# kubernetes-sigs/lws

Hardware: AMD Instinct MI355X
Metric: replica-group time-to-ready + rollout p50; Llama-3-70B 1-leader/0-worker TP=1 (lower is better)
Workload: dtype bf16; 1 GPU; model=llama-3-70b, global_batch=32, seq_len=128, parallelism=tp1, group=1-leader/0-workers (size=1), replicas=1, collectives_staged=False, orchestrator=lws_amd in-process control plane

## Files before the change

### lws_amd/models/llama.py

```python
from __future__ import annotations

import math
from dataclasses import dataclass
import torch

from ..parallel.tp import ShardedLinear, all_gather_cat, all_reduce


@dataclass
class LlamaConfig:
    name: str = "llama"
    hidden_size: int = 4096
    intermediate_size: int = 14336
    num_layers: int = 32
    num_q_heads: int = 32
    num_kv_heads: int = 8
    head_dim: int = 128
    vocab_size: int = 128256
    rope_theta: float = 500000.0
    rms_eps: float = 1e-5
    max_position: int = 8192
    num_experts: int = 0
    num_experts_per_tok: int = 2

    @property
    def q_size(self) -> int:
        return self.num_q_heads * self.head_dim

    @property
    def kv_size(self) -> int:
        return self.num_kv_heads * self.head_dim

    def num_params(self) -> int:
        h, i, v = self.hidden_size, self.intermediate_size, self.vocab_size
        mlp = 3 * h * i
        if self.num_experts > 0:
            mlp = self.num_experts * 3 * h * i + h * self.num_experts
        per_layer = (h * self.q_size + 2 * h * self.kv_size + self.q_size * h
                     + mlp + 2 * h)
        return self.num_layers * per_layer + 2 * v * h + h


def llama3_8b() -> LlamaConfig:
    return LlamaConfig(name="llama-3-8b", hidden_size=4096,
                       intermediate_size=14336, num_layers=32, num_q_heads=32,
                       num_kv_heads=8, vocab_size=128256)


def llama3_70b() -> LlamaConfig:
    return LlamaConfig(name="llama-3-70b", hidden_size=8192,
                       intermediate_size=28672, num_layers=80, num_q_heads=64,
                       num_kv_heads=8, vocab_size=128256)


def mixtral_8x7b() -> LlamaConfig:
    return LlamaConfig(name="mixtral-8x7b", hidden_size=4096,
                       intermediate_size=14336, num_layers=32, num_q_heads=32,
                       num_kv_heads=8, vocab_size=32000, rope_theta=1e6,
                       num_experts=8, num_experts_per_tok=2)


def mixtral_tiny() -> LlamaConfig:
    return LlamaConfig(name="mixtral-tiny", hidden_size=256,
                       intermediate_size=512, num_layers=2, num_q_heads=8,
                       num_kv_heads=2, head_dim=128, vocab_size=1024,
                       max_position=2048, num_experts=4,
                       num_experts_per_tok=2)


def llama_tiny() -> LlamaConfig:
    return LlamaConfig(name="llama-tiny", hidden_size=256,
                       intermediate_size=512, num_layers=2, num_q_heads=8,
                       num_kv_heads=2, head_dim=128, vocab_size=1024,
                       max_position=2048)


def llama_tiny8() -> LlamaConfig:
    return LlamaConfig(name="llama-tiny8", hidden_size=256,
                       intermediate_size=512, num_layers=2, num_q_heads=8,
                       num_kv_heads=8, head_dim=128, vocab_size=1024,
                       max_position=2048)


def llama_tiny4() -> LlamaConfig:
    return LlamaConfig(name="llama-tiny4", hidden_size=256,
                       intermediate_size=512, num_layers=2, num_q_heads=8,
# ... 76 lines not shown
                w0 = lins[0].weight
                stacked = torch.empty(cfg.num_experts, *w0.shape,
                                      device=device, dtype=dtype)
                for i, lin in enumerate(lins):
                    lin.weight = stacked[i]
                return stacked
            self.experts_gate_up_w = stack(self.experts_gate_up)
            self.experts_down_w = stack(self.experts_down)
            self.gate_up = None
            self.down = None
        else:
            self.router = None
            self.gate_up = ShardedLinear(2 * cfg.intermediate_size, h, 0,
                                         tp_rank, tp_world, device, dtype)
            self.down = ShardedLinear(h, cfg.intermediate_size, 1, tp_rank,
                                      tp_world, device, dtype)
        self.input_norm = torch.empty(h, device=device, dtype=dtype)
        self.post_norm = torch.empty(h, device=device, dtype=dtype)
        self.q_slice = self.hq * d
        self.kv_slice = self.hkv * d

    def materialize(self, gen=None):
        lins = [self.qkv, self.o]
        if self.router is not None:
            self.router.normal_(0.0, 0.02, generator=gen)
            lins += self.experts_gate_up + self.experts_down
        else:
            lins += [self.gate_up, self.down]
        for lin in lins:
            lin.materialize(gen)
        self.input_norm.fill_(1.0)
        self.post_norm.fill_(1.0)

    @property
    def param_count(self) -> int:
        n = self.qkv.numel + self.o.numel
        n += self.input_norm.numel() + self.post_norm.numel()
        if self.router is not None:
            n += self.router.numel()
            n += sum(l.numel for l in self.experts_gate_up)
            n += sum(l.numel for l in self.experts_down)
        else:
            n += self.gate_up.numel + self.down.numel
        return n


class LlamaForCausalLM:
    def __init__(self, cfg: LlamaConfig, tp_rank: int = 0, tp_world: int = 1,
                 device: str = "cpu", dtype=torch.bfloat16,
                 pp_rank: int = 0, pp_world: int = 1):
        self.cfg = cfg
        self.tp_rank = tp_rank
        self.tp_world = tp_world
        self.pp_rank = pp_rank
        self.pp_world = pp_world
        assert tp_world == 1 or pp_world == 1, \
            "combined TP x PP grids are not supported"
        self.device = torch.device(device)
        self.dtype = dtype
        self._ops = _Ops(self.device)
        L, base, rem = cfg.num_layers, cfg.num_layers // pp_world, \
            cfg.num_layers % pp_world
        sizes = [base + (1 if r < rem else 0) for r in range(pp_world)]
        self.layer_offset = sum(sizes[:pp_rank])
        self.pp_first = pp_rank == 0
        self.pp_last = pp_rank == pp_world - 1
        self.layers = [LlamaLayer(cfg, tp_rank, tp_world, self.device, dtype)
                       for _ in range(sizes[pp_rank])]
        self.embed = torch.empty(cfg.vocab_size, cfg.hidden_size,
                                 device=self.device, dtype=dtype) \
            if self.pp_first else None
        self.final_norm = torch.empty(cfg.hidden_size, device=self.device,
                                      dtype=dtype) if self.pp_last else None
        self.lm_head = ShardedLinear(cfg.vocab_size, cfg.hidden_size, 0,
                                     tp_rank, tp_world, self.device, dtype) \
            if self.pp_last else None
        from lws_amd.ops import build_rope_table
        self.rope_table = build_rope_table(cfg.max_position, cfg.head_dim,
                                           cfg.rope_theta, device=self.device)
        self.scale = 1.0 / math.sqrt(cfg.head_dim)
        self._ar = all_reduce if tp_world > 1 else (lambda t: t)
        self._agc = all_gather_cat if tp_world > 1 \
            else (lambda t, dim=-1: t)

    def materialize(self, seed: int = 0) -> int:
        def gen_for(tag: int) -> torch.Generator:
            g = torch.Generator(device=self.device)
            g.manual_seed(seed * 1000003 + tag * 7919 + self.tp_rank)
            return g
        n = 0
        for i, layer in enumerate(self.layers):
            layer.materialize(gen_for(self.layer_offset + i))
            n += layer.param_count
        if self.embed is not None:
            self.embed.normal_(0.0, 0.02, generator=gen_for(500009))
            n += self.embed.numel()
        if self.final_norm is not None:
            self.final_norm.fill_(1.0)
            n += self.final_norm.numel()
        if self.lm_head is not None:
            self.lm_head.materialize(gen_for(600011))
            n += self.lm_head.numel
        return n

    def quantize_fp8(self) -> None:
        for layer in self.layers:
            lins = [layer.qkv, layer.o]
            if layer.router is None:
                lins += [layer.gate_up, layer.down]
            for lin in lins:
                lin.quantize_fp8()
            if layer.router is not None:
                for name, lins in (
                        ("experts_gate_up_w", layer.experts_gate_up),
                        ("experts_down_w", layer.experts_down)):
                    w = getattr(layer, name)
                    sc = (w.abs().amax(dim=2).float() / 448.0) \
                        .clamp(min=1e-8).contiguous()
                    w8 = (w.float() / sc[:, :, None]).clamp(-448.0, 448.0) \
                        .to(torch.float8_e4m3fn).contiguous()
                    setattr(layer, name + "8", w8)
                    setattr(layer, name + "_scale", sc)
                    setattr(layer, name, None)
                    for e, lin in enumerate(lins):
                        lin.weight_fp8 = w8[e]
                        lin.scale_fp8 = sc[e]
                        lin.weight = None
        if self.lm_head is not None:
            self.lm_head.quantize_fp8()

    def kv_cache_spec(self) -> tuple[int, int]:
        return len(self.layers), self.layers[0].hkv

    def _rmsnorm(self, x, w):
        if self._ops.is_gpu:
            return self._ops.ops.rmsnorm(x, w, self.cfg.rms_eps)
        return self._ops.ref.rmsnorm_ref(x, w, self.cfg.rms_eps)

    def _fused_add_rmsnorm(self, x, residual, w):
        if self._ops.is_gpu:
            self._ops.ops.fused_add_rmsnorm(x, residual, w, self.cfg.rms_eps)
            return x, residual
        out, new_res = self._ops.ref.fused_add_rmsnorm_ref(
            x, residual, w, self.cfg.rms_eps)
        return out, new_res

    def _silu_mul(self, gu):
        if self._ops.is_gpu:
            return self._ops.ops.silu_mul(gu)
        return self._ops.ref.silu_mul_ref(gu)

    def _write_cache(self, k, v, k_cache, v_cache, slot_mapping):
        if self._ops.is_gpu:
            self._ops.ops.reshape_and_cache(k, v, k_cache, v_cache, slot_mapping)
            return
        page = k_cache.size(2)
        for t in range(k.size(0)):
            s = int(slot_mapping[t])
            if s < 0:
                continue
            k_cache[s // page, :, s % page] = k[t]
            v_cache[s // page, :, s % page] = v[t]

    def _qkv_views(self, qkv: torch.Tensor, layer, positions):
        d = self.cfg.head_dim
        if self._ops.is_gpu:
            q = qkv.narrow(-1, 0, layer.q_slice).unflatten(-1, (layer.hq, d))
            k = qkv.narrow(-1, layer.q_slice,
                           layer.kv_slice).unflatten(-1, (layer.hkv, d))
            v = qkv.narrow(-1, layer.q_slice + layer.kv_slice,
                           layer.kv_slice).unflatten(-1, (layer.hkv, d))
            self._ops.ops.rope(q, k, self.rope_table, positions,
                               layer.hq, layer.hkv)
            return q, k, v
        q, k, v = qkv.split([layer.q_slice, layer.kv_slice, layer.kv_slice],
                            dim=-1)
        q, k = self._ops.ref.rope_ref(q.contiguous(), k.contiguous(),
                                      self.rope_table, positions,
                                      layer.hq, layer.hkv)
        T = qkv.size(0)
        return (q.view(T, layer.hq, d), k.view(T, layer.hkv, d),
                v.contiguous().view(T, layer.hkv, d))

    def forward_prefill(self, batch: PrefillBatch, kv_caches) -> torch.Tensor:
        cfg = self.cfg
        if self.pp_first:
            x = self.embed[batch.input_ids]
            residual = None
        else:
            from ..parallel import pp as ppmod
            T = batch.input_ids.size(0)
            st = ppmod.recv_stage((2, T, cfg.hidden_size), self.dtype,
                                  self.device, self.pp_rank - 1)
            x, residual = st[0], st[1]
        for li, layer in enumerate(self.layers):
            if residual is None:
                residual = x
                h = self._rmsnorm(x, layer.input_norm)
            else:
                h, residual = self._fused_add_rmsnorm(x, residual,
                                                      layer.input_norm)
            qkv = layer.qkv(h)
            q, k, v = self._qkv_views(qkv, layer, batch.positions)
            k_cache, v_cache = kv_caches[li]
            self._write_cache(k, v, k_cache, v_cache, batch.slot_mapping)
            attn = self._prefill_attention(q, k, v, batch, layer,
                                           k_cache, v_cache)
            o = layer.o(attn)
            x = self._ar(o)
            h, residual = self._fused_add_rmsnorm(x, residual, layer.post_norm)
            x = self._ar(self._mlp(layer, h))
        B = len(batch.seq_starts) - 1
        if not self.pp_last:
            from ..parallel import pp as ppmod
            ppmod.send_stage(torch.stack([x, residual]), self.pp_rank + 1)
            return torch.zeros(B, self.cfg.hidden_size, device=self.device,
                               dtype=self.dtype)
        h, _ = self._fused_add_rmsnorm(x, residual, self.final_norm)
        last = torch.tensor([s - 1 for s in batch.seq_starts[1:]],
                            device=h.device, dtype=torch.long)
        return h[last]

    def _prefill_attention(self, q, k, v, batch: PrefillBatch, layer,
                           k_cache, v_cache):
        cfg = self.cfg
        d = cfg.head_dim
        kv_starts = batch.seq_starts
        q_offsets = None
        if batch.kv_row_idx is not None:
            k = k_cache.reshape(-1, d).index_select(
                0, batch.kv_row_idx).view(-1, layer.hkv, d)
            v = v_cache.reshape(-1, d).index_select(
                0, batch.kv_row_idx).view(-1, layer.hkv, d)
            kv_starts = batch.kv_starts
            q_offsets = batch.q_offsets
        if self._ops.is_gpu:
            return self._ops.ops.prefill_attention(
                q, k, v, batch.seq_starts, self.scale,
                kv_starts=kv_starts, q_offsets=q_offsets)
        T = q.size(0)
        out = torch.empty(T, layer.hq * d, device=q.device, dtype=q.dtype)
        G = layer.hq // layer.hkv
        offs = q_offsets or [0] * (len(batch.seq_starts) - 1)
        for i in range(len(batch.seq_starts) - 1):
            s0, s1 = batch.seq_starts[i], batch.seq_starts[i + 1]
            kv0, kv1 = kv_starts[i], kv_starts[i + 1]
            S, KV, off = s1 - s0, kv1 - kv0, offs[i]
            qs = q[s0:s1].transpose(0, 1)
            ks = k[kv0:kv1].transpose(0, 1)
            vs = v[kv0:kv1].transpose(0, 1)
            ks = ks.repeat_interleave(G, dim=0)
            vs = vs.repeat_interleave(G, dim=0)
            scores = (qs @ ks.transpose(-1, -2)).float() * self.scale
            cols = torch.arange(KV, device=q.device)
            rows = torch.arange(S, device=q.device)
            mask = torch.where(cols[None, :] > off + rows[:, None],
                               float("-inf"), 0.0)
            p = torch.softmax(scores + mask, dim=-1).to(q.dtype)
            o = (p @ vs).transpose(0, 1).reshape(S, layer.hq * d)
            out[s0:s1] = o
        return out

    def forward_decode(self, batch: DecodeBatch, kv_caches) -> torch.Tensor:
        cfg = self.cfg
        if self.pp_first:
            x = self.embed[batch.input_ids]
            residual = None
        else:
            from ..parallel import pp as ppmod
            B0 = batch.input_ids.size(0)
            st = ppmod.recv_stage((2, B0, cfg.hidden_size), self.dtype,
                                  self.device, self.pp_rank - 1)
            x, residual = st[0], st[1]
        fp8q = (self._ops.is_gpu and self.layers
                and getattr(self.layers[0].qkv, "weight_fp8", None)
                is not None and self.layers[0].router is None
                and x.size(0) <= 32 and cfg.hidden_size % 256 == 0
                and self.layers[0].down.weight_fp8.size(1) % 256 == 0)
        for li, layer in enumerate(self.layers):
            if fp8q:
                if residual is None:
                    residual = x
                    h8, hs = self._ops.ops.rmsnorm_fp8(x, layer.input_norm,
                                                       cfg.rms_eps)
                else:
                    h8, hs = self._ops.ops.fused_add_rmsnorm_fp8(
                        x, residual, layer.input_norm, cfg.rms_eps)
                qkv = layer.qkv.forward_q8(h8, hs)
            else:
                if residual is None:
                    residual = x
                    h = self._rmsnorm(x, layer.input_norm)
                else:
                    h, residual = self._fused_add_rmsnorm(x, residual,
                                                          layer.input_norm)
                qkv = layer.qkv(h)
            k_cache, v_cache = kv_caches[li]
            if self._ops.is_gpu:
                d = cfg.head_dim
                q = qkv.narrow(-1, 0, layer.q_slice) \
                    .unflatten(-1, (layer.hq, d))
                k = qkv.narrow(-1, layer.q_slice, layer.kv_slice) \
                    .unflatten(-1, (layer.hkv, d))
                vv = qkv.narrow(-1, layer.q_slice + layer.kv_slice,
                                layer.kv_slice).unflatten(-1, (layer.hkv, d))
                self._ops.ops.rope_and_cache(q, k, vv, self.rope_table,
                                             batch.positions, k_cache,
                                             v_cache, batch.slot_mapping)
            else:
                q, k, v = self._qkv_views(qkv, layer, batch.positions)
                self._write_cache(k, v, k_cache, v_cache,
                                  batch.slot_mapping)
            B = q.size(0)
            if self._ops.is_gpu:
                attn = self._ops.ops.paged_attention_decode(
                    q, k_cache, v_cache, batch.block_tables, batch.seq_lens,
                    self.scale)
            else:
                attn = self._ops.ref.paged_attention_decode_ref(
                    q.contiguous(), k_cache, v_cache, batch.block_tables,
                    batch.seq_lens, self.scale)
            o = layer.o(attn.view(B, layer.hq * cfg.head_dim))
            x = self._ar(o)
            if fp8q:
                h8, hs = self._ops.ops.fused_add_rmsnorm_fp8(
                    x, residual, layer.post_norm, cfg.rms_eps)
                gu = layer.gate_up.forward_q8(h8, hs)
                a8, ascale = self._ops.ops.silu_mul_fp8(gu)
                x = self._ar(layer.down.forward_q8(a8, ascale))
            else:
                h, residual = self._fused_add_rmsnorm(x, residual,
                                                      layer.post_norm)
                x = self._ar(self._mlp(layer, h))
        if not self.pp_last:
            from ..parallel import pp as ppmod
            ppmod.send_stage(torch.stack([x, residual]), self.pp_rank + 1)
            return torch.zeros_like(x)
        h, _ = self._fused_add_rmsnorm(x, residual, self.final_norm)
        return h

    def _mlp(self, layer, h: torch.Tensor) -> torch.Tensor:
        if layer.router is None:
            return layer.down(self._silu_mul(layer.gate_up(h)))
        cfg = self.cfg
        logits = (h.float() @ layer.router.float().t())
        weights, chosen = torch.topk(torch.softmax(logits, dim=-1),
                                     cfg.num_experts_per_tok, dim=-1)
        weights = weights / weights.sum(dim=-1, keepdim=True)
        out = torch.zeros_like(h)
        if self._ops.is_gpu and h.size(0) <= 32:
            E = cfg.num_experts
            T = h.size(0)
            tk = cfg.num_experts_per_tok
            flat = chosen.reshape(-1)
            oh = torch.nn.functional.one_hot(flat, E)
            ranks = oh.cumsum(0) - oh
            rank_sel = ranks.gather(1, flat.unsqueeze(1)).squeeze(1)
            dest = flat * T + rank_sel
            tok = torch.arange(T, device=h.device).repeat_interleave(tk)
            x_pad = torch.zeros(E * T, h.size(1), dtype=h.dtype,
                                device=h.device)
            x_pad.index_copy_(0, dest, h.index_select(0, tok))
# ... 37 lines not shown
```

### lws_amd/ops/__init__.py

```python
from __future__ import annotations

from pathlib import Path
from typing import Optional

import torch

_LIB = None
_LOAD_ERROR: Optional[str] = None


def _try_load() -> None:
    global _LIB, _LOAD_ERROR
    if _LIB is not None or _LOAD_ERROR is not None:
        return
    so = Path(__file__).resolve().parent / "_C.so"
    if not so.exists():
        _LOAD_ERROR = f"{so} not built (run python -m lws_amd.ops.build)"
        return
    try:
        torch.ops.load_library(str(so))
    except Exception:
        pass
    try:
        import importlib.util

        spec = importlib.util.spec_from_file_location("lws_amd_C", str(so))
        mod = importlib.util.module_from_spec(spec)
        spec.loader.exec_module(mod)
        _LIB = mod
    except Exception as e:
        _LOAD_ERROR = f"failed to load {so}: {e}"


def native_available() -> bool:
    _try_load()
    return _LIB is not None


def require_native():
    _try_load()
    if _LIB is None:
        raise RuntimeError(
            "lws_amd native kernels unavailable on a GPU host: "
            f"{_LOAD_ERROR}. Build with `python -m lws_amd.ops.build`.")
    return _LIB



def rmsnorm(x: torch.Tensor, weight: torch.Tensor, eps: float = 1e-5,
            out: Optional[torch.Tensor] = None) -> torch.Tensor:
    lib = require_native()
    if out is None:
        out = torch.empty_like(x)
    lib.rmsnorm(out, x, weight, eps)
    return out


def fused_add_rmsnorm(x: torch.Tensor, residual: torch.Tensor,
                      weight: torch.Tensor, eps: float = 1e-5) -> None:
    lib = require_native()
    lib.fused_add_rmsnorm(x, residual, weight, eps)


def silu_mul(gateup: torch.Tensor,
             out: Optional[torch.Tensor] = None) -> torch.Tensor:
    lib = require_native()
    shape = list(gateup.shape)
    shape[-1] //= 2
    if out is None:
        out = torch.empty(shape, dtype=gateup.dtype, device=gateup.device)
    lib.silu_mul(out, gateup)
    return out


def rope(q: torch.Tensor, k: torch.Tensor, cos_sin: torch.Tensor,
         positions: torch.Tensor, num_q_heads: int, num_kv_heads: int) -> None:
    lib = require_native()
    lib.rope(q, k, cos_sin, positions, num_q_heads, num_kv_heads)


def rope_and_cache(q, k, v, cos_sin, positions, k_cache, v_cache,
                   slot_mapping) -> None:
    lib = require_native()
    lib.rope_and_cache(q, k, v, cos_sin, positions, k_cache, v_cache,
                       slot_mapping)


def build_rope_table(max_pos: int, head_dim: int, theta: float = 10000.0,
                     device="cpu") -> torch.Tensor:
    half = head_dim // 2
    inv_freq = 1.0 / (theta ** (torch.arange(0, half, dtype=torch.float64) / half))
    pos = torch.arange(max_pos, dtype=torch.float64)
    ang = torch.outer(pos, inv_freq)
    table = torch.cat([torch.cos(ang), torch.sin(ang)], dim=-1).float()
    return table.to(device)


_PA_WS: dict = {}


def paged_attention_decode(q: torch.Tensor, k_cache: torch.Tensor,
                           v_cache: torch.Tensor, block_tables: torch.Tensor,
                           seq_lens: torch.Tensor, scale: float,
                           chunk_keys: Optional[int] = None,
                           workspace: Optional[tuple] = None,
                           out: Optional[torch.Tensor] = None) -> torch.Tensor:
    import os as _os

    lib = require_native()
    B, Hq, D = q.shape
    Hkv = k_cache.size(1)
    G = Hq // Hkv
    mfma = G in (4, 8, 16) and _os.environ.get("LWS_PA_MFMA", "1") != "0"
    max_len = int(block_tables.size(1)) * int(k_cache.size(2))
    if chunk_keys is None:
        if B * Hkv >= 256 and G == 1 and max_len <= 512:
            chunk_keys = ((max_len + 15) // 16) * 16
        else:
            if B * Hkv <= 64:
                if mfma:
                    target_chunks = max(1, min(8, -(-max_len // 64)))
                else:
                    target_chunks = min(16, (max_len + 31) // 32)
            else:
                target_chunks = max(1, min(4, -(-max_len // 96)))
            chunk_keys = -(-max_len // target_chunks)
            chunk_keys = ((chunk_keys + 15) // 16) * 16
    num_chunks = max(1, (max_len + chunk_keys - 1) // chunk_keys)
    if mfma:
        num_chunks *= 4
    if workspace is None:
        key = ("paws", B, Hkv, num_chunks, G, q.device.index)
        ws = _PA_WS.get(key)
        if ws is None:
            ws = (torch.empty((B, Hkv, num_chunks, G, D),
                              dtype=torch.float32, device=q.device),
                  torch.empty((B, Hkv, num_chunks, G, 2),
                              dtype=torch.float32, device=q.device))
            _PA_WS[key] = ws
        ws_acc, ws_ml = ws
    else:
        ws_acc, ws_ml = workspace
        num_chunks = ws_ml.size(2)
    if out is None:
        out = torch.empty_like(q)
    lib.paged_attention_decode(out, q, k_cache, v_cache, block_tables,
                               seq_lens, ws_acc, ws_ml, scale, chunk_keys)
    return out


def reshape_and_cache(k: torch.Tensor, v: torch.Tensor, k_cache: torch.Tensor,
                      v_cache: torch.Tensor, slot_mapping: torch.Tensor) -> None:
    lib = require_native()
    lib.reshape_and_cache(k, v, k_cache, v_cache, slot_mapping)


SKINNY_GEMM_MAX_M = 32
_SKINNY_WS: dict = {}


def skinny_gemm(x: torch.Tensor, w: torch.Tensor,
                out: Optional[torch.Tensor] = None) -> torch.Tensor:
    lib = require_native()
    grouped = x.dim() == 3
    E = x.size(0) if grouped else 1
    M, K = x.shape[-2], x.shape[-1]
    N = w.size(-2)
    if out is None:
        shape = (E, M, N) if grouped else (M, N)
        out = torch.empty(shape, dtype=x.dtype, device=x.device)
    import os
    target = int(os.environ.get("LWS_SG_TARGET", "256"))
    n_blocks = (N + 63) // 64
    split = min(max(1, target // max(1, n_blocks)), max(1, K // 128))
    k_slice = (K // split + 127) // 128 * 128
    grid_y = (K + k_slice - 1) // k_slice
    if grouped and E * n_blocks >= 256:
        grid_y = 1
    key = (grid_y, E, M, N, x.device.index)
    ws = _SKINNY_WS.get(key)
    if ws is None:
        ws = torch.empty(grid_y, E * M, N, dtype=torch.float32,
                         device=x.device)
        _SKINNY_WS[key] = ws
    lib.skinny_gemm(out, x, w, ws)
    return out


_SKINNY_FP8_BUFS: dict = {}


def skinny_gemm_fp8(x: torch.Tensor, w8: torch.Tensor, w_scale: torch.Tensor,
                    out: Optional[torch.Tensor] = None) -> torch.Tensor:
    lib = require_native()
    M, K = x.shape
    N = w8.size(0)
    if out is None:
        out = torch.empty(M, N, dtype=torch.bfloat16, device=x.device)
    import os
    target = int(os.environ.get("LWS_SG8_TARGET", "512"))
    ksub = int(os.environ.get("LWS_SG8_KSUB", "128"))
    rows = 32 if (os.environ.get("LWS_SG8_ROWS") == "32"
                  and ksub == 128) else 64
    n_blocks = (N + rows - 1) // rows
    split = min(max(1, target // max(1, n_blocks)), max(1, K // ksub))
    k_slice = (K // split + ksub - 1) // ksub * ksub
    grid_y = (K + k_slice - 1) // k_slice
    key = (grid_y, M, N, K, x.device.index)
    bufs = _SKINNY_FP8_BUFS.get(key)
    if bufs is None:
        bufs = (torch.empty(M, K, dtype=torch.float8_e4m3fn, device=x.device),
                torch.empty(M, dtype=torch.float32, device=x.device),
                torch.empty(grid_y, M, N, dtype=torch.float32,
                            device=x.device))
        _SKINNY_FP8_BUFS[key] = bufs
    x8, xs, ws = bufs
    lib.quant_fp8_rows(x8, xs, x.contiguous())
    lib.skinny_gemm_fp8(out, x8, xs, w8, w_scale, ws)
    return out


def skinny_gemm_fp8_grouped(x: torch.Tensor, w8: torch.Tensor,
                            w_scale: torch.Tensor,
                            out: Optional[torch.Tensor] = None
                            ) -> torch.Tensor:
    lib = require_native()
    E, M, K = x.shape
    N = w8.size(1)
    if out is None:
        out = torch.empty(E, M, N, dtype=torch.bfloat16, device=x.device)
    key = ("g8", E, M, N, K, x.device.index)
    bufs = _SKINNY_FP8_BUFS.get(key)
    if bufs is None:
        bufs = (torch.empty(E, M, K, dtype=torch.float8_e4m3fn,
                            device=x.device),
                torch.empty(E, M, dtype=torch.float32, device=x.device),
                torch.empty(1, M, N, dtype=torch.float32, device=x.device))
        _SKINNY_FP8_BUFS[key] = bufs
    x8, xs, ws = bufs
    lib.quant_fp8_rows(x8.view(E * M, K), xs.view(E * M), x.reshape(E * M, K))
    lib.skinny_gemm_fp8(out, x8, xs, w8, w_scale, ws)
    return out


def skinny_gemm_fp8_q(x8: torch.Tensor, xs: torch.Tensor, w8: torch.Tensor,
                      w_scale: torch.Tensor,
                      out: Optional[torch.Tensor] = None) -> torch.Tensor:
    lib = require_native()
    M, K = x8.shape
    N = w8.size(0)
    if out is None:
        out = torch.empty(M, N, dtype=torch.bfloat16, device=x8.device)
    import os
    target = int(os.environ.get("LWS_SG8_TARGET", "512"))
    ksub = int(os.environ.get("LWS_SG8_KSUB", "128"))
    rows = 32 if (os.environ.get("LWS_SG8_ROWS") == "32"
                  and ksub == 128) else 64
    n_blocks = (N + rows - 1) // rows
    split = min(max(1, target // max(1, n_blocks)), max(1, K // ksub))
    k_slice = (K // split + ksub - 1) // ksub * ksub
    grid_y = (K + k_slice - 1) // k_slice
    key = ("q8ws", grid_y, M, N, x8.device.index)
    ws = _SKINNY_FP8_BUFS.get(key)
    if ws is None:
        ws = torch.empty(grid_y, M, N, dtype=torch.float32, device=x8.device)
        _SKINNY_FP8_BUFS[key] = ws
    lib.skinny_gemm_fp8(out, x8, xs, w8, w_scale, ws)
    return out


_FP8_ACT_BUFS: dict = {}


def _fp8_act_buffers(rows: int, cols: int, device) -> tuple:
    key = (rows, cols, device.index if device.type == "cuda" else -1)
    bufs = _FP8_ACT_BUFS.get(key)
    if bufs is None:
        bufs = (torch.empty(rows, cols, dtype=torch.float8_e4m3fn,
                            device=device),
                torch.empty(rows, dtype=torch.float32, device=device))
        _FP8_ACT_BUFS[key] = bufs
    return bufs


def rmsnorm_fp8(x: torch.Tensor, weight: torch.Tensor,
                eps: float = 1e-5) -> tuple:
    lib = require_native()
    rows, D = x.shape[0], x.shape[-1]
    y8, ys = _fp8_act_buffers(rows, D, x.device)
    lib.rmsnorm_fp8(y8, ys, x.contiguous(), weight, eps)
    return y8, ys


def fused_add_rmsnorm_fp8(x: torch.Tensor, residual: torch.Tensor,
                          weight: torch.Tensor, eps: float = 1e-5) -> tuple:
    lib = require_native()
    rows, D = x.shape[0], x.shape[-1]
    y8, ys = _fp8_act_buffers(rows, D, x.device)
    lib.fused_add_rmsnorm_fp8(y8, ys, x.contiguous(), residual, weight, eps)
    return y8, ys


def silu_mul_fp8(gateup: torch.Tensor) -> tuple:
    lib = require_native()
    rows = gateup.shape[0]
    I = gateup.shape[-1] // 2
    a8, ascale = _fp8_act_buffers(rows, I, gateup.device)
    lib.silu_mul_fp8(a8, ascale, gateup.contiguous())
    return a8, ascale


def prefill_attention(q: torch.Tensor, k: torch.Tensor, v: torch.Tensor,
                      seq_starts: list, scale: float,
                      out: Optional[torch.Tensor] = None,
                      kv_starts: Optional[list] = None,
                      q_offsets: Optional[list] = None) -> torch.Tensor:
    lib = require_native()
    T, Hq, D = q.shape
    device = q.device
    B = len(seq_starts) - 1
    tile_seq, tile_q0 = [], []
    for i in range(B):
        S = seq_starts[i + 1] - seq_starts[i]
        for q0 in range(0, S, 64):
            tile_seq.append(i)
            tile_q0.append(q0)
    if kv_starts is None:
        kv_starts = seq_starts
    if q_offsets is None:
        q_offsets = [0] * B
    if out is None:
        out = torch.empty(T, Hq * D, dtype=q.dtype, device=device)
    lib.prefill_attention(
        out, q, k, v,
        torch.tensor(tile_seq, dtype=torch.int32, device=device),
        torch.tensor(tile_q0, dtype=torch.int32, device=device),
        torch.tensor(seq_starts, dtype=torch.int32, device=device),
        torch.tensor(kv_starts, dtype=torch.int32, device=device),
        torch.tensor(q_offsets, dtype=torch.int32, device=device), scale)
    return out
```

### lws_amd/ops/build.py

```python
from __future__ import annotations

import os
import shutil
import sys
from pathlib import Path

PKG_DIR = Path(__file__).resolve().parent
CSRC = PKG_DIR / "csrc"
SO_NAME = "_C.so"
SOURCES = ["norm_act.hip", "rope.hip", "paged_attention.hip",
           "skinny_gemm.hip", "skinny_gemm_fp8.hip", "prefill_attention.hip",
           "bindings.cpp"]


def _newest_source_mtime() -> float:
    return max((CSRC / s).stat().st_mtime for s in SOURCES) if CSRC.exists() else 0


def needs_build() -> bool:
    so = PKG_DIR / SO_NAME
    if not so.exists():
        return True
    return so.stat().st_mtime < _newest_source_mtime()


def build(verbose: bool = False, force: bool = False) -> Path:
    so_path = PKG_DIR / SO_NAME
    if not force and not needs_build():
        return so_path

    os.environ.setdefault("PYTORCH_ROCM_ARCH", "gfx950")
    from torch.utils.cpp_extension import load

    build_dir = PKG_DIR / "build"
    build_dir.mkdir(exist_ok=True)
    load(
        name="lws_amd_C",
        sources=[str(CSRC / s) for s in SOURCES],
        extra_cflags=["-O3", "-std=c++17"],
        extra_cuda_cflags=["-O3", "-std=c++17"],
        build_directory=str(build_dir),
        verbose=verbose,
        is_python_module=True,
        keep_intermediates=True,
    )
    built = build_dir / "lws_amd_C.so"
    if not built.exists():
        raise RuntimeError(f"extension build produced no {built}")
    shutil.copy2(built, so_path)
    return so_path


if __name__ == "__main__":
    p = build(verbose="-v" in sys.argv, force="-f" in sys.argv)
    print(f"built {p}")
```

### lws_amd/ops/csrc/bindings.cpp

```cpp
#include <torch/extension.h>

void rmsnorm(torch::Tensor out, torch::Tensor input, torch::Tensor weight,
             double eps);
void fused_add_rmsnorm(torch::Tensor x, torch::Tensor residual,
                       torch::Tensor weight, double eps);
void silu_mul(torch::Tensor out, torch::Tensor gateup);
void rmsnorm_fp8(torch::Tensor out8, torch::Tensor oscale,
                 torch::Tensor input, torch::Tensor weight, double eps);
void fused_add_rmsnorm_fp8(torch::Tensor out8, torch::Tensor oscale,
                           torch::Tensor x, torch::Tensor residual,
                           torch::Tensor weight, double eps);
void silu_mul_fp8(torch::Tensor out8, torch::Tensor oscale,
                  torch::Tensor gateup);
void rope(torch::Tensor q, torch::Tensor k, torch::Tensor cos_sin,
          torch::Tensor positions, long long num_q_heads,
          long long num_kv_heads);
void rope_and_cache(torch::Tensor q, torch::Tensor k, torch::Tensor v,
                    torch::Tensor cos_sin, torch::Tensor positions,
                    torch::Tensor k_cache, torch::Tensor v_cache,
                    torch::Tensor slot_mapping);
void paged_attention_decode(torch::Tensor out, torch::Tensor q,
                            torch::Tensor k_cache, torch::Tensor v_cache,
                            torch::Tensor block_tables, torch::Tensor seq_lens,
                            torch::Tensor ws_acc, torch::Tensor ws_ml,
                            double scale, long long chunk_keys);
void reshape_and_cache(torch::Tensor k, torch::Tensor v,
                       torch::Tensor k_cache, torch::Tensor v_cache,
                       torch::Tensor slot_mapping);
void skinny_gemm(torch::Tensor out, torch::Tensor x, torch::Tensor w,
                 torch::Tensor ws);
void skinny_gemm_fp8(torch::Tensor out, torch::Tensor x8, torch::Tensor xs,
                     torch::Tensor w8, torch::Tensor ws_n, torch::Tensor ws);
void quant_fp8_rows(torch::Tensor x8, torch::Tensor xs, torch::Tensor x);
void prefill_attention(torch::Tensor out, torch::Tensor q, torch::Tensor k,
                       torch::Tensor v, torch::Tensor tile_seq,
                       torch::Tensor tile_q0, torch::Tensor seq_starts,
                       torch::Tensor kv_starts, torch::Tensor q_offs,
                       double scale);

PYBIND11_MODULE(TORCH_EXTENSION_NAME, m) {
  m.def("rmsnorm", &rmsnorm, "RMSNorm (bf16, gfx950)");
  m.def("fused_add_rmsnorm", &fused_add_rmsnorm,
        "in-place residual add + RMSNorm (bf16, gfx950)");
  m.def("silu_mul", &silu_mul, "fused SiLU-gate multiply (bf16, gfx950)");
  m.def("rmsnorm_fp8", &rmsnorm_fp8,
        "RMSNorm with fused per-token e4m3 quantization epilogue");
  m.def("fused_add_rmsnorm_fp8", &fused_add_rmsnorm_fp8,
        "residual add + RMSNorm with fused e4m3 quantization epilogue");
  m.def("silu_mul_fp8", &silu_mul_fp8,
        "SiLU-gate multiply with fused e4m3 quantization epilogue");
  m.def("rope", &rope, "fused rotary embedding for q,k (bf16, gfx950)");
  m.def("rope_and_cache", &rope_and_cache,
        "rope on q in place + rotated k and v scattered into the paged "
        "KV cache (single decode launch)");
  m.def("paged_attention_decode", &paged_attention_decode,
        "GQA paged attention decode with flash-decoding chunk split");
  m.def("reshape_and_cache", &reshape_and_cache,
        "scatter new k/v into the paged KV cache");
  m.def("skinny_gemm", &skinny_gemm,
        "split-K MFMA GEMM for decode-shape projections (M<=32)");
  m.def("skinny_gemm_fp8", &skinny_gemm_fp8,
        "W8A8 e4m3 split-K MFMA GEMM for decode projections (M<=32)");
  m.def("quant_fp8_rows", &quant_fp8_rows,
        "per-token e4m3 activation quantization (bf16 -> fp8 + scales)");
  m.def("prefill_attention", &prefill_attention,
        "flash-style causal varlen prefill attention (GQA, gfx950)");
}
```

### lws_amd/parallel/tp.py

```python
from __future__ import annotations

import os
from dataclasses import dataclass
from typing import Optional

import torch
import torch.distributed as dist


@dataclass
class ParallelState:
    rank: int = 0
    world_size: int = 1
    local_rank: int = 0
    device: torch.device = torch.device("cpu")
    group: Optional[object] = None
    staged: bool = False

    @property
    def is_distributed(self) -> bool:
        return self.world_size > 1


_STATE = ParallelState()
# ... 32 lines not shown
    return _STATE


def all_reduce(t: torch.Tensor) -> torch.Tensor:
    if _STATE.is_distributed and dist.is_initialized():
        if _STATE.staged and t.is_cuda:
            host = t.detach().to("cpu")
            dist.all_reduce(host)
            t.copy_(host)
        else:
            dist.all_reduce(t)
    return t


def all_gather_cat(t: torch.Tensor, dim: int = -1) -> torch.Tensor:
    if not (_STATE.is_distributed and dist.is_initialized()):
        return t
    if _STATE.staged and t.is_cuda:
        host = t.detach().contiguous().to("cpu")
        parts = [torch.empty_like(host) for _ in range(_STATE.world_size)]
        dist.all_gather(parts, host)
        return torch.cat(parts, dim=dim).to(t.device)
    parts = [torch.empty_like(t) for _ in range(_STATE.world_size)]
    dist.all_gather(parts, t.contiguous())
    return torch.cat(parts, dim=dim)


def barrier() -> None:
    if _STATE.is_distributed and dist.is_initialized():
        dist.barrier()



class ShardedLinear:

    def __init__(self, out_features: int, in_features: int, shard_dim: int,
                 tp_rank: int, tp_world: int, device, dtype=torch.bfloat16):
        self.shard_dim = shard_dim
        if shard_dim == 0:
            assert out_features % tp_world == 0
            shape = (out_features // tp_world, in_features)
        else:
            assert in_features % tp_world == 0
            shape = (out_features, in_features // tp_world)
        self.weight = torch.empty(shape, device=device, dtype=dtype)
        self.weight_fp8: Optional[torch.Tensor] = None
        self.scale_fp8: Optional[torch.Tensor] = None
        self._ones: Optional[torch.Tensor] = None

    def materialize(self, generator: Optional[torch.Generator] = None,
                    std: float = 0.02) -> None:
        self.weight.normal_(0.0, std, generator=generator)

    def quantize_fp8(self) -> None:
        w = self.weight
        self.scale_fp8 = (w.abs().amax(dim=1).float() / 448.0) \
            .clamp(min=1e-8).contiguous()
        self.weight_fp8 = (w.float() / self.scale_fp8[:, None]).clamp(
            -448.0, 448.0).to(torch.float8_e4m3fn).contiguous()
        self.weight = None

    def __call__(self, x: torch.Tensor) -> torch.Tensor:
        if self.weight_fp8 is not None:
            M = x.size(0)
            if not x.is_cuda:
                wf = self.weight_fp8.float() * self.scale_fp8[:, None]
                return (x.float() @ wf.t()).to(torch.bfloat16)
            if x.dim() == 2 and M <= 32 and x.size(1) % 256 == 0:
                from .. import ops
                return ops.skinny_gemm_fp8(x, self.weight_fp8,
                                           self.scale_fp8)
            pad = (-M) % 16
            if pad:
                x = torch.nn.functional.pad(x, (0, 0, 0, pad))
            xs = (x.abs().amax().float() / 448.0).clamp(min=1e-8)
            x8 = (x.float() / xs).clamp(-448.0, 448.0).to(torch.float8_e4m3fn)
            if self._ones is None or self._ones.device != x.device:
                self._ones = torch.ones((), device=x.device)
            out = torch._scaled_mm(x8, self.weight_fp8.t(), scale_a=xs,
                                   scale_b=self._ones,
                                   out_dtype=torch.bfloat16)
            out = out * self.scale_fp8.to(torch.bfloat16)[None, :]
            return out[:M] if pad else out
        if x.is_cuda and x.dim() == 2 and x.size(0) <= 32 and \
                x.size(1) % 128 == 0 and self._skinny_wins():
            from .. import ops
            return ops.skinny_gemm(x.contiguous(), self.weight)
        return x @ self.weight.t()

    def _skinny_wins(self) -> bool:
        N, K = self.weight.shape
        if N * K <= 32 * 1024 * 1024:
            return True
        if K <= 4096:
            return True
        if K >= 16384 and N >= 8192:
            return True
        return False

    def forward_q8(self, x8: torch.Tensor, xs: torch.Tensor) -> torch.Tensor:
        from .. import ops
        return ops.skinny_gemm_fp8_q(x8, xs, self.weight_fp8, self.scale_fp8)

    @property
    def numel(self) -> int:
        w = self.weight if self.weight is not None else self.weight_fp8
        return w.numel()
```

Baseline: 287.1 ms.

## Move per-layer attention and MLP sequencing into native C++ block ops

Adds C++ entry points (decode_attn_block, prefill_attn_block, mlp_block) that run norm, QKV projection, rope/cache write, attention and output projection inside one native call per block. GEMM workspaces, the paged-attention plan and the prefill attention metadata tensors are now computed once per forward instead of once per layer. The aim is to cut Python dispatch and repeated host-to-device metadata tensor creation. It also adds a tightened N%16 condition for skinny GEMM and a new native path that has to stay numerically consistent with the Python path.

```diff
diff --git a/lws_amd/models/llama.py b/lws_amd/models/llama.py
--- a/lws_amd/models/llama.py
+++ b/lws_amd/models/llama.py
@@ -2,6 +2,8 @@
 
 import math
 from dataclasses import dataclass
+from typing import Optional
+
 import torch
 
 from ..parallel.tp import ShardedLinear, all_gather_cat, all_reduce
@@ -244,6 +246,19 @@
         self._ar = all_reduce if tp_world > 1 else (lambda t: t)
         self._agc = all_gather_cat if tp_world > 1 \
             else (lambda t, dim=-1: t)
+        self._native_blocks: Optional[bool] = None
+
+    @property
+    def native_blocks(self) -> bool:
+        if self._native_blocks is False:
+            return False
+        return (self._ops.is_gpu and bool(self.layers)
+                and self.layers[0].router is None
+                and self.layers[0].qkv.weight_fp8 is None)
+
+    @native_blocks.setter
+    def native_blocks(self, value: bool) -> None:
+        self._native_blocks = bool(value)
 
     def materialize(self, seed: int = 0) -> int:
         def gen_for(tag: int) -> torch.Generator:
@@ -355,7 +370,36 @@
             st = ppmod.recv_stage((2, T, cfg.hidden_size), self.dtype,
                                   self.device, self.pp_rank - 1)
             x, residual = st[0], st[1]
+        meta = None
+        if self._ops.is_gpu:
+            chunked = batch.kv_row_idx is not None
+            meta = self._ops.ops.prefill_attention_meta(
+                batch.seq_starts, batch.kv_starts if chunked else None,
+                batch.q_offsets if chunked else None, x.device)
+        native = self.native_blocks
+        if native:
+            lib = self._ops.ops.require_native()
+            T = x.size(0)
+            l0 = self.layers[0]
+            qkv_ws, o_ws = l0.qkv.plan(T), l0.o.plan(T)
+            gate_up_ws, down_ws = l0.gate_up.plan(T), l0.down.plan(T)
         for li, layer in enumerate(self.layers):
+            if native:
+                k_cache, v_cache = kv_caches[li]
+                o = lib.prefill_attn_block(
+                    x, residual, layer.input_norm, cfg.rms_eps,
+                    layer.qkv.weight, qkv_ws, layer.o.weight, o_ws,
+                    self.rope_table, batch.positions, k_cache, v_cache,
+                    batch.slot_mapping, batch.kv_row_idx, *meta, self.scale,
+                    layer.hq, layer.hkv)
+                if residual is None:
+                    residual = x
+                x = self._ar(o)
+                x = self._ar(lib.mlp_block(
+                    x, residual, layer.post_norm, cfg.rms_eps,
+                    layer.gate_up.weight, gate_up_ws, layer.down.weight,
+                    down_ws))
+                continue
             if residual is None:
                 residual = x
                 h = self._rmsnorm(x, layer.input_norm)
@@ -367,7 +411,7 @@
             k_cache, v_cache = kv_caches[li]
             self._write_cache(k, v, k_cache, v_cache, batch.slot_mapping)
             attn = self._prefill_attention(q, k, v, batch, layer,
-                                           k_cache, v_cache)
+                                           k_cache, v_cache, meta)
             o = layer.o(attn)
             x = self._ar(o)
             h, residual = self._fused_add_rmsnorm(x, residual, layer.post_norm)
@@ -384,7 +428,7 @@
         return h[last]
 
     def _prefill_attention(self, q, k, v, batch: PrefillBatch, layer,
-                           k_cache, v_cache):
+                           k_cache, v_cache, meta=None):
         cfg = self.cfg
         d = cfg.head_dim
         kv_starts = batch.seq_starts
@@ -399,7 +443,7 @@
         if self._ops.is_gpu:
             return self._ops.ops.prefill_attention(
                 q, k, v, batch.seq_starts, self.scale,
-                kv_starts=kv_starts, q_offsets=q_offsets)
+                kv_starts=kv_starts, q_offsets=q_offsets, meta=meta)
         T = q.size(0)
         out = torch.empty(T, layer.hq * d, device=q.device, dtype=q.dtype)
         G = layer.hq // layer.hkv
@@ -439,7 +483,35 @@
                 is not None and self.layers[0].router is None
                 and x.size(0) <= 32 and cfg.hidden_size % 256 == 0
                 and self.layers[0].down.weight_fp8.size(1) % 256 == 0)
+        native = self.native_blocks
+        if native:
+            lib = self._ops.ops.require_native()
+            B = x.size(0)
+            l0 = self.layers[0]
+            page_size = kv_caches[0][0].size(2)
+            chunk_keys, ws_acc, ws_ml = self._ops.ops.paged_attention_plan(
+                B, l0.hq, l0.hkv, cfg.head_dim,
+                int(batch.block_tables.size(1)) * int(page_size), x.device)
+            qkv_ws, o_ws = l0.qkv.plan(B), l0.o.plan(B)
+            gate_up_ws, down_ws = l0.gate_up.plan(B), l0.down.plan(B)
         for li, layer in enumerate(self.layers):
+            if native:
+                k_cache, v_cache = kv_caches[li]
+                o = lib.decode_attn_block(
+                    x, residual, layer.input_norm, cfg.rms_eps,
+                    layer.qkv.weight, qkv_ws, layer.o.weight, o_ws,
+                    self.rope_table, batch.positions, k_cache, v_cache,
+                    batch.slot_mapping, batch.block_tables, batch.seq_lens,
+                    ws_acc, ws_ml, self.scale, chunk_keys, layer.hq,
+                    layer.hkv)
+                if residual is None:
+                    residual = x
+                x = self._ar(o)
+                x = self._ar(lib.mlp_block(
+                    x, residual, layer.post_norm, cfg.rms_eps,
+                    layer.gate_up.weight, gate_up_ws, layer.down.weight,
+                    down_ws))
+                continue
             if fp8q:
                 if residual is None:
                     residual = x
diff --git a/lws_amd/ops/__init__.py b/lws_amd/ops/__init__.py
--- a/lws_amd/ops/__init__.py
+++ b/lws_amd/ops/__init__.py
@@ -99,20 +99,12 @@
 _PA_WS: dict = {}
 
 
-def paged_attention_decode(q: torch.Tensor, k_cache: torch.Tensor,
-                           v_cache: torch.Tensor, block_tables: torch.Tensor,
-                           seq_lens: torch.Tensor, scale: float,
-                           chunk_keys: Optional[int] = None,
-                           workspace: Optional[tuple] = None,
-                           out: Optional[torch.Tensor] = None) -> torch.Tensor:
+def paged_attention_chunk_policy(B: int, Hq: int, Hkv: int, max_len: int,
+                                 chunk_keys: Optional[int] = None) -> tuple:
     import os as _os
 
-    lib = require_native()
-    B, Hq, D = q.shape
-    Hkv = k_cache.size(1)
     G = Hq // Hkv
     mfma = G in (4, 8, 16) and _os.environ.get("LWS_PA_MFMA", "1") != "0"
-    max_len = int(block_tables.size(1)) * int(k_cache.size(2))
     if chunk_keys is None:
         if B * Hkv >= 256 and G == 1 and max_len <= 512:
             chunk_keys = ((max_len + 15) // 16) * 16
@@ -129,19 +121,43 @@
     num_chunks = max(1, (max_len + chunk_keys - 1) // chunk_keys)
     if mfma:
         num_chunks *= 4
+    return chunk_keys, num_chunks
+
+
+def paged_attention_plan(B: int, Hq: int, Hkv: int, D: int, max_len: int,
+                         device, chunk_keys: Optional[int] = None) -> tuple:
+    chunk_keys, num_chunks = paged_attention_chunk_policy(
+        B, Hq, Hkv, max_len, chunk_keys)
+    G = Hq // Hkv
+    device = torch.device(device)
+    key = ("paws", B, Hkv, num_chunks, G, device.index)
+    ws = _PA_WS.get(key)
+    if ws is None:
+        ws = (torch.empty((B, Hkv, num_chunks, G, D),
+                          dtype=torch.float32, device=device),
+              torch.empty((B, Hkv, num_chunks, G, 2),
+                          dtype=torch.float32, device=device))
+        _PA_WS[key] = ws
+    return chunk_keys, ws[0], ws[1]
+
+
+def paged_attention_decode(q: torch.Tensor, k_cache: torch.Tensor,
+                           v_cache: torch.Tensor, block_tables: torch.Tensor,
+                           seq_lens: torch.Tensor, scale: float,
+                           chunk_keys: Optional[int] = None,
+                           workspace: Optional[tuple] = None,
+                           out: Optional[torch.Tensor] = None) -> torch.Tensor:
+    lib = require_native()
+    B, Hq, D = q.shape
+    Hkv = k_cache.size(1)
+    max_len = int(block_tables.size(1)) * int(k_cache.size(2))
     if workspace is None:
-        key = ("paws", B, Hkv, num_chunks, G, q.device.index)
-        ws = _PA_WS.get(key)
-        if ws is None:
-            ws = (torch.empty((B, Hkv, num_chunks, G, D),
-                              dtype=torch.float32, device=q.device),
-                  torch.empty((B, Hkv, num_chunks, G, 2),
-                              dtype=torch.float32, device=q.device))
-            _PA_WS[key] = ws
-        ws_acc, ws_ml = ws
+        chunk_keys, ws_acc, ws_ml = paged_attention_plan(
+            B, Hq, Hkv, D, max_len, q.device, chunk_keys)
     else:
+        if chunk_keys is None:
+            chunk_keys, _ = paged_attention_chunk_policy(B, Hq, Hkv, max_len)
         ws_acc, ws_ml = workspace
-        num_chunks = ws_ml.size(2)
     if out is None:
         out = torch.empty_like(q)
     lib.paged_attention_decode(out, q, k_cache, v_cache, block_tables,
@@ -159,30 +175,45 @@
 _SKINNY_WS: dict = {}
 
 
-def skinny_gemm(x: torch.Tensor, w: torch.Tensor,
-                out: Optional[torch.Tensor] = None) -> torch.Tensor:
-    lib = require_native()
-    grouped = x.dim() == 3
-    E = x.size(0) if grouped else 1
-    M, K = x.shape[-2], x.shape[-1]
-    N = w.size(-2)
-    if out is None:
-        shape = (E, M, N) if grouped else (M, N)
-        out = torch.empty(shape, dtype=x.dtype, device=x.device)
+def skinny_gemm_split(E: int, N: int, K: int,
+                      grouped: Optional[bool] = None) -> int:
     import os
     target = int(os.environ.get("LWS_SG_TARGET", "256"))
     n_blocks = (N + 63) // 64
     split = min(max(1, target // max(1, n_blocks)), max(1, K // 128))
     k_slice = (K // split + 127) // 128 * 128
     grid_y = (K + k_slice - 1) // k_slice
+    if grouped is None:
+        grouped = E > 1
     if grouped and E * n_blocks >= 256:
         grid_y = 1
-    key = (grid_y, E, M, N, x.device.index)
+    return grid_y
+
+
+def skinny_gemm_workspace(E: int, M: int, N: int, K: int, device,
+                          grouped: Optional[bool] = None) -> torch.Tensor:
+    grid_y = skinny_gemm_split(E, N, K, grouped)
+    device = torch.device(device)
+    key = (grid_y, E, M, N, device.index)
     ws = _SKINNY_WS.get(key)
     if ws is None:
         ws = torch.empty(grid_y, E * M, N, dtype=torch.float32,
-                         device=x.device)
+                         device=device)
         _SKINNY_WS[key] = ws
+    return ws
+
+
+def skinny_gemm(x: torch.Tensor, w: torch.Tensor,
+                out: Optional[torch.Tensor] = None) -> torch.Tensor:
+    lib = require_native()
+    grouped = x.dim() == 3
+    E = x.size(0) if grouped else 1
+    M, K = x.shape[-2], x.shape[-1]
+    N = w.size(-2)
+    if out is None:
+        shape = (E, M, N) if grouped else (M, N)
+        out = torch.empty(shape, dtype=x.dtype, device=x.device)
+    ws = skinny_gemm_workspace(E, M, N, K, x.device, grouped)
     lib.skinny_gemm(out, x, w, ws)
     return out
 
@@ -310,14 +341,8 @@
     return a8, ascale
 
 
-def prefill_attention(q: torch.Tensor, k: torch.Tensor, v: torch.Tensor,
-                      seq_starts: list, scale: float,
-                      out: Optional[torch.Tensor] = None,
-                      kv_starts: Optional[list] = None,
-                      q_offsets: Optional[list] = None) -> torch.Tensor:
-    lib = require_native()
-    T, Hq, D = q.shape
-    device = q.device
+def prefill_attention_meta(seq_starts: list, kv_starts: Optional[list],
+                           q_offsets: Optional[list], device) -> tuple:
     B = len(seq_starts) - 1
     tile_seq, tile_q0 = [], []
     for i in range(B):
@@ -329,13 +354,25 @@
         kv_starts = seq_starts
     if q_offsets is None:
         q_offsets = [0] * B
-    if out is None:
-        out = torch.empty(T, Hq * D, dtype=q.dtype, device=device)
-    lib.prefill_attention(
-        out, q, k, v,
-        torch.tensor(tile_seq, dtype=torch.int32, device=device),
-        torch.tensor(tile_q0, dtype=torch.int32, device=device),
-        torch.tensor(seq_starts, dtype=torch.int32, device=device),
-        torch.tensor(kv_starts, dtype=torch.int32, device=device),
-        torch.tensor(q_offsets, dtype=torch.int32, device=device), scale)
-    return out
+    return (torch.tensor(tile_seq, dtype=torch.int32, device=device),
+            torch.tensor(tile_q0, dtype=torch.int32, device=device),
+            torch.tensor(seq_starts, dtype=torch.int32, device=device),
+            torch.tensor(kv_starts, dtype=torch.int32, device=device),
+            torch.tensor(q_offsets, dtype=torch.int32, device=device))
+
+
+def prefill_attention(q: torch.Tensor, k: torch.Tensor, v: torch.Tensor,
+                      seq_starts: list, scale: float,
+                      out: Optional[torch.Tensor] = None,
+                      kv_starts: Optional[list] = None,
+                      q_offsets: Optional[list] = None,
+                      meta: Optional[tuple] = None) -> torch.Tensor:
+    lib = require_native()
+    T, Hq, D = q.shape
+    if meta is None:
+        meta = prefill_attention_meta(seq_starts, kv_starts, q_offsets,
+                                      q.device)
+    if out is None:
+        out = torch.empty(T, Hq * D, dtype=q.dtype, device=q.device)
+    lib.prefill_attention(out, q, k, v, *meta, scale)
+    return out
diff --git a/lws_amd/ops/build.py b/lws_amd/ops/build.py
--- a/lws_amd/ops/build.py
+++ b/lws_amd/ops/build.py
@@ -10,11 +10,14 @@
 SO_NAME = "_C.so"
 SOURCES = ["norm_act.hip", "rope.hip", "paged_attention.hip",
            "skinny_gemm.hip", "skinny_gemm_fp8.hip", "prefill_attention.hip",
-           "bindings.cpp"]
+           "layer_blocks.cpp", "bindings.cpp"]
+HEADERS = ["common.h", "launchers.h"]
 
 
 def _newest_source_mtime() -> float:
-    return max((CSRC / s).stat().st_mtime for s in SOURCES) if CSRC.exists() else 0
+    if not CSRC.exists():
+        return 0
+    return max((CSRC / s).stat().st_mtime for s in SOURCES + HEADERS)
 
 
 def needs_build() -> bool:
diff --git a/lws_amd/ops/csrc/bindings.cpp b/lws_amd/ops/csrc/bindings.cpp
--- a/lws_amd/ops/csrc/bindings.cpp
+++ b/lws_amd/ops/csrc/bindings.cpp
@@ -1,42 +1,7 @@
 #include <torch/extension.h>
+#include <pybind11/stl.h>
 
-void rmsnorm(torch::Tensor out, torch::Tensor input, torch::Tensor weight,
-             double eps);
-void fused_add_rmsnorm(torch::Tensor x, torch::Tensor residual,
-                       torch::Tensor weight, double eps);
-void silu_mul(torch::Tensor out, torch::Tensor gateup);
-void rmsnorm_fp8(torch::Tensor out8, torch::Tensor oscale,
-                 torch::Tensor input, torch::Tensor weight, double eps);
-void fused_add_rmsnorm_fp8(torch::Tensor out8, torch::Tensor oscale,
-                           torch::Tensor x, torch::Tensor residual,
-                           torch::Tensor weight, double eps);
-void silu_mul_fp8(torch::Tensor out8, torch::Tensor oscale,
-                  torch::Tensor gateup);
-void rope(torch::Tensor q, torch::Tensor k, torch::Tensor cos_sin,
-          torch::Tensor positions, long long num_q_heads,
-          long long num_kv_heads);
-void rope_and_cache(torch::Tensor q, torch::Tensor k, torch::Tensor v,
-                    torch::Tensor cos_sin, torch::Tensor positions,
-                    torch::Tensor k_cache, torch::Tensor v_cache,
-                    torch::Tensor slot_mapping);
-void paged_attention_decode(torch::Tensor out, torch::Tensor q,
-                            torch::Tensor k_cache, torch::Tensor v_cache,
-                            torch::Tensor block_tables, torch::Tensor seq_lens,
-                            torch::Tensor ws_acc, torch::Tensor ws_ml,
-                            double scale, long long chunk_keys);
-void reshape_and_cache(torch::Tensor k, torch::Tensor v,
-                       torch::Tensor k_cache, torch::Tensor v_cache,
-                       torch::Tensor slot_mapping);
-void skinny_gemm(torch::Tensor out, torch::Tensor x, torch::Tensor w,
-                 torch::Tensor ws);
-void skinny_gemm_fp8(torch::Tensor out, torch::Tensor x8, torch::Tensor xs,
-                     torch::Tensor w8, torch::Tensor ws_n, torch::Tensor ws);
-void quant_fp8_rows(torch::Tensor x8, torch::Tensor xs, torch::Tensor x);
-void prefill_attention(torch::Tensor out, torch::Tensor q, torch::Tensor k,
-                       torch::Tensor v, torch::Tensor tile_seq,
-                       torch::Tensor tile_q0, torch::Tensor seq_starts,
-                       torch::Tensor kv_starts, torch::Tensor q_offs,
-                       double scale);
+#include "launchers.h"
 
 PYBIND11_MODULE(TORCH_EXTENSION_NAME, m) {
   m.def("rmsnorm", &rmsnorm, "RMSNorm (bf16, gfx950)");
@@ -65,4 +30,15 @@
         "per-token e4m3 activation quantization (bf16 -> fp8 + scales)");
   m.def("prefill_attention", &prefill_attention,
         "flash-style causal varlen prefill attention (GQA, gfx950)");
+  m.def("decode_attn_block", &decode_attn_block,
+        py::call_guard<py::gil_scoped_release>(),
+        "decode: input norm, qkv GEMM, rope_and_cache, paged attention, "
+        "o-proj GEMM (returns the pre-all-reduce o-proj output)");
+  m.def("prefill_attn_block", &prefill_attn_block,
+        py::call_guard<py::gil_scoped_release>(),
+        "prefill: input norm, qkv GEMM, rope, reshape_and_cache, optional "
+        "cache gather, prefill attention, o-proj GEMM");
+  m.def("mlp_block", &mlp_block, py::call_guard<py::gil_scoped_release>(),
+        "fused_add_rmsnorm, gate_up GEMM, silu_mul, down GEMM (returns the "
+        "pre-all-reduce result)");
 }
diff --git a/lws_amd/ops/csrc/launchers.h b/lws_amd/ops/csrc/launchers.h
--- /dev/null
+++ b/lws_amd/ops/csrc/launchers.h
@@ -0,0 +1,66 @@
+#pragma once
+
+#include <torch/extension.h>
+
+void rmsnorm(torch::Tensor out, torch::Tensor input, torch::Tensor weight,
+             double eps);
+void fused_add_rmsnorm(torch::Tensor x, torch::Tensor residual,
+                       torch::Tensor weight, double eps);
+void silu_mul(torch::Tensor out, torch::Tensor gateup);
+void rmsnorm_fp8(torch::Tensor out8, torch::Tensor oscale,
+                 torch::Tensor input, torch::Tensor weight, double eps);
+void fused_add_rmsnorm_fp8(torch::Tensor out8, torch::Tensor oscale,
+                           torch::Tensor x, torch::Tensor residual,
+                           torch::Tensor weight, double eps);
+void silu_mul_fp8(torch::Tensor out8, torch::Tensor oscale,
+                  torch::Tensor gateup);
+void rope(torch::Tensor q, torch::Tensor k, torch::Tensor cos_sin,
+          torch::Tensor positions, long long num_q_heads,
+          long long num_kv_heads);
+void rope_and_cache(torch::Tensor q, torch::Tensor k, torch::Tensor v,
+                    torch::Tensor cos_sin, torch::Tensor positions,
+                    torch::Tensor k_cache, torch::Tensor v_cache,
+                    torch::Tensor slot_mapping);
+void paged_attention_decode(torch::Tensor out, torch::Tensor q,
+                            torch::Tensor k_cache, torch::Tensor v_cache,
+                            torch::Tensor block_tables, torch::Tensor seq_lens,
+                            torch::Tensor ws_acc, torch::Tensor ws_ml,
+                            double scale, long long chunk_keys);
+void reshape_and_cache(torch::Tensor k, torch::Tensor v,
+                       torch::Tensor k_cache, torch::Tensor v_cache,
+                       torch::Tensor slot_mapping);
+void skinny_gemm(torch::Tensor out, torch::Tensor x, torch::Tensor w,
+                 torch::Tensor ws);
+void skinny_gemm_fp8(torch::Tensor out, torch::Tensor x8, torch::Tensor xs,
+                     torch::Tensor w8, torch::Tensor ws_n, torch::Tensor ws);
+void quant_fp8_rows(torch::Tensor x8, torch::Tensor xs, torch::Tensor x);
+void prefill_attention(torch::Tensor out, torch::Tensor q, torch::Tensor k,
+                       torch::Tensor v, torch::Tensor tile_seq,
+                       torch::Tensor tile_q0, torch::Tensor seq_starts,
+                       torch::Tensor kv_starts, torch::Tensor q_offs,
+                       double scale);
+
+torch::Tensor decode_attn_block(
+    torch::Tensor x, std::optional<torch::Tensor> residual,
+    torch::Tensor input_norm, double eps, torch::Tensor qkv_w,
+    std::optional<torch::Tensor> qkv_ws, torch::Tensor o_w,
+    std::optional<torch::Tensor> o_ws, torch::Tensor cos_sin,
+    torch::Tensor positions, torch::Tensor k_cache, torch::Tensor v_cache,
+    torch::Tensor slot_mapping, torch::Tensor block_tables,
+    torch::Tensor seq_lens, torch::Tensor ws_acc, torch::Tensor ws_ml,
+    double scale, long long chunk_keys, long long hq, long long hkv);
+torch::Tensor prefill_attn_block(
+    torch::Tensor x, std::optional<torch::Tensor> residual,
+    torch::Tensor input_norm, double eps, torch::Tensor qkv_w,
+    std::optional<torch::Tensor> qkv_ws, torch::Tensor o_w,
+    std::optional<torch::Tensor> o_ws, torch::Tensor cos_sin,
+    torch::Tensor positions, torch::Tensor k_cache, torch::Tensor v_cache,
+    torch::Tensor slot_mapping, std::optional<torch::Tensor> kv_row_idx,
+    torch::Tensor tile_seq, torch::Tensor tile_q0, torch::Tensor seq_starts,
+    torch::Tensor kv_starts, torch::Tensor q_offs, double scale,
+    long long hq, long long hkv);
+torch::Tensor mlp_block(
+    torch::Tensor x, torch::Tensor residual, torch::Tensor post_norm,
+    double eps, torch::Tensor gate_up_w,
+    std::optional<torch::Tensor> gate_up_ws, torch::Tensor down_w,
+    std::optional<torch::Tensor> down_ws);
diff --git a/lws_amd/ops/csrc/layer_blocks.cpp b/lws_amd/ops/csrc/layer_blocks.cpp
--- /dev/null
+++ b/lws_amd/ops/csrc/layer_blocks.cpp
@@ -0,0 +1,114 @@
+#include "launchers.h"
+
+#include <ATen/ATen.h>
+
+namespace {
+
+constexpr int64_t kSkinnyMaxM = 32;
+constexpr int64_t kSkinnyKSub = 128;
+
+torch::Tensor project(const torch::Tensor& x, const torch::Tensor& w,
+                      const std::optional<torch::Tensor>& ws) {
+  const int64_t M = x.size(0), K = x.size(1), N = w.size(0);
+  if (ws.has_value() && ws->defined() && M <= kSkinnyMaxM &&
+      K % kSkinnyKSub == 0 && N % 16 == 0) {
+    torch::Tensor out = at::empty({M, N}, x.options());
+    skinny_gemm(out, x.contiguous(), w, *ws);
+    return out;
+  }
+  return at::mm(x, w.t());
+}
+
+torch::Tensor input_norm_step(torch::Tensor& x,
+                              const std::optional<torch::Tensor>& residual,
+                              const torch::Tensor& weight, double eps) {
+  if (!residual.has_value() || !residual->defined()) {
+    torch::Tensor h = at::empty_like(x);
+    rmsnorm(h, x, weight, eps);
+    return h;
+  }
+  fused_add_rmsnorm(x, *residual, weight, eps);
+  return x;
+}
+
+struct QKV {
+  torch::Tensor q, k, v;
+};
+
+QKV split_qkv(const torch::Tensor& qkv, int64_t hq, int64_t hkv) {
+  const int64_t total = qkv.size(-1);
+  TORCH_CHECK(hq > 0 && hkv > 0 && total % (hq + 2 * hkv) == 0,
+              "qkv width does not match the head counts");
+  const int64_t d = total / (hq + 2 * hkv);
+  const int64_t qs = hq * d, kvs = hkv * d;
+  return {qkv.narrow(-1, 0, qs).unflatten(-1, {hq, d}),
+          qkv.narrow(-1, qs, kvs).unflatten(-1, {hkv, d}),
+          qkv.narrow(-1, qs + kvs, kvs).unflatten(-1, {hkv, d})};
+}
+
+}
+
+torch::Tensor decode_attn_block(
+    torch::Tensor x, std::optional<torch::Tensor> residual,
+    torch::Tensor input_norm, double eps, torch::Tensor qkv_w,
+    std::optional<torch::Tensor> qkv_ws, torch::Tensor o_w,
+    std::optional<torch::Tensor> o_ws, torch::Tensor cos_sin,
+    torch::Tensor positions, torch::Tensor k_cache, torch::Tensor v_cache,
+    torch::Tensor slot_mapping, torch::Tensor block_tables,
+    torch::Tensor seq_lens, torch::Tensor ws_acc, torch::Tensor ws_ml,
+    double scale, long long chunk_keys, long long hq, long long hkv) {
+  TORCH_CHECK(x.dim() == 2, "decode_attn_block: x must be [B, H]");
+  torch::Tensor h = input_norm_step(x, residual, input_norm, eps);
+  torch::Tensor qkv = project(h, qkv_w, qkv_ws);
+  QKV s = split_qkv(qkv, hq, hkv);
+  rope_and_cache(s.q, s.k, s.v, cos_sin, positions, k_cache, v_cache,
+                 slot_mapping);
+  const int64_t B = s.q.size(0), d = s.q.size(2);
+  torch::Tensor attn = at::empty({B, hq, d}, s.q.options());
+  paged_attention_decode(attn, s.q, k_cache, v_cache, block_tables, seq_lens,
+                         ws_acc, ws_ml, scale, chunk_keys);
+  return project(attn.view({B, hq * d}), o_w, o_ws);
+}
+
+torch::Tensor prefill_attn_block(
+    torch::Tensor x, std::optional<torch::Tensor> residual,
+    torch::Tensor input_norm, double eps, torch::Tensor qkv_w,
+    std::optional<torch::Tensor> qkv_ws, torch::Tensor o_w,
+    std::optional<torch::Tensor> o_ws, torch::Tensor cos_sin,
+    torch::Tensor positions, torch::Tensor k_cache, torch::Tensor v_cache,
+    torch::Tensor slot_mapping, std::optional<torch::Tensor> kv_row_idx,
+    torch::Tensor tile_seq, torch::Tensor tile_q0, torch::Tensor seq_starts,
+    torch::Tensor kv_starts, torch::Tensor q_offs, double scale,
+    long long hq, long long hkv) {
+  TORCH_CHECK(x.dim() == 2, "prefill_attn_block: x must be [T, H]");
+  torch::Tensor h = input_norm_step(x, residual, input_norm, eps);
+  torch::Tensor qkv = project(h, qkv_w, qkv_ws);
+  QKV s = split_qkv(qkv, hq, hkv);
+  rope(s.q, s.k, cos_sin, positions, hq, hkv);
+  reshape_and_cache(s.k, s.v, k_cache, v_cache, slot_mapping);
+  const int64_t T = s.q.size(0), d = s.q.size(2);
+  torch::Tensor k = s.k, v = s.v;
+  if (kv_row_idx.has_value() && kv_row_idx->defined()) {
+    k = k_cache.reshape({-1, d}).index_select(0, *kv_row_idx)
+            .view({-1, hkv, d});
+    v = v_cache.reshape({-1, d}).index_select(0, *kv_row_idx)
+            .view({-1, hkv, d});
+  }
+  torch::Tensor attn = at::empty({T, hq * d}, s.q.options());
+  prefill_attention(attn, s.q, k, v, tile_seq, tile_q0, seq_starts, kv_starts,
+                    q_offs, scale);
+  return project(attn, o_w, o_ws);
+}
+
+torch::Tensor mlp_block(
+    torch::Tensor x, torch::Tensor residual, torch::Tensor post_norm,
+    double eps, torch::Tensor gate_up_w,
+    std::optional<torch::Tensor> gate_up_ws, torch::Tensor down_w,
+    std::optional<torch::Tensor> down_ws) {
+  TORCH_CHECK(x.dim() == 2, "mlp_block: x must be [T, H]");
+  fused_add_rmsnorm(x, residual, post_norm, eps);
+  torch::Tensor gu = project(x, gate_up_w, gate_up_ws);
+  torch::Tensor act = at::empty({gu.size(0), gu.size(1) / 2}, gu.options());
+  silu_mul(act, gu);
+  return project(act, down_w, down_ws);
+}
diff --git a/lws_amd/parallel/tp.py b/lws_amd/parallel/tp.py
--- a/lws_amd/parallel/tp.py
+++ b/lws_amd/parallel/tp.py
@@ -138,14 +138,31 @@
                                    out_dtype=torch.bfloat16)
             out = out * self.scale_fp8.to(torch.bfloat16)[None, :]
             return out[:M] if pad else out
-        if x.is_cuda and x.dim() == 2 and x.size(0) <= 32 and \
-                x.size(1) % 128 == 0 and self._skinny_wins():
+        if x.dim() == 2 and self.plan(x.size(0)) is not None:
             from .. import ops
             return ops.skinny_gemm(x.contiguous(), self.weight)
         return x @ self.weight.t()
 
-    def _skinny_wins(self) -> bool:
+    def uses_skinny(self, M: int) -> bool:
+        w = self.weight
+        if w is None or not w.is_cuda:
+            return False
+        return self.skinny_rule(M, w.size(0), w.size(1))
+
+    @staticmethod
+    def skinny_rule(M: int, N: int, K: int) -> bool:
+        return (M <= 32 and K % 128 == 0 and N % 16 == 0
+                and ShardedLinear._skinny_wins(N, K))
+
+    def plan(self, M: int) -> Optional[torch.Tensor]:
+        if not self.uses_skinny(M):
+            return None
+        from .. import ops
         N, K = self.weight.shape
+        return ops.skinny_gemm_workspace(1, M, N, K, self.weight.device)
+
+    @staticmethod
+    def _skinny_wins(N: int, K: int) -> bool:
         if N * K <= 32 * 1024 * 1024:
             return True
         if K <= 4096:
```

Result: faster. 190.4 ms, median of 6 (-33.7%).
